# lifthrasiir/j40

Measured on AMD Instinct MI355X. Metric: Mpixels/s RGBA-u8x4 decode, 8K VarDCT d1, higher is better.
Workload: dtype f32

## Files before the change

j40_amd/csrc/device/async.hip:

```cpp
#include <hip/hip_runtime.h>
#include <chrono>
#include <cstdio>
#include <memory>
#include <mutex>
#include <vector>
#include "../decode_route.hpp"
#include "../plan_front.hpp"
#include "kernels.h"
#include "runtime_shared.hpp"
#include "hostcopy.hpp"
#include "async.hpp"

using namespace j40hip;
using namespace j40hip_rt;

namespace {

constexpr uint32_t ERR_GPU = ('!' << 24) | ('g' << 16) | ('p' << 8) | 'u';
constexpr uint32_t ERR_MEM = ('!' << 24) | ('m' << 16) | ('e' << 8) | 'm';

struct StaticEntry {
	int device = 0;
	std::vector<uint8_t> key;
	uint32_t order_off[11 * 13 * 3], dq_off[17], dq_size[17], dq_scan_off[17];
// ... 482 lines not shown
	}
	if ((size_t) n * 4 + 16 > b->verdict_cap) {
		if (b->verdict_host) (void) hipHostFree(b->verdict_host);
		b->verdict_host = nullptr; b->verdict_cap = 0;
		if (hipHostMalloc((void **) &b->verdict_host, 16 * (size_t) n * 2 + 64, hipHostMallocDefault) != hipSuccess) { (void) hipGetLastError(); return ERR_MEM; }
		b->verdict_cap = (size_t) n * 4 * 2 + 16;
	}
	uint8_t *hb = b->host.ptr, *db = (uint8_t *) b->dev;
	b->last_o_k2 = o_k2;
	DevPlan *h_plans = (DevPlan *) (hb + o_plans); DevPlanBuild *h_builds = (DevPlanBuild *) (hb + o_builds); K2Frame *h_k2 = (K2Frame *) (hb + o_k2);
	DevBatchLf *h_lfs = (DevBatchLf *) (hb + o_lfs);
	const DevPlan *d_plans = (const DevPlan *) (db + o_plans); const DevPlanBuild *d_builds = (const DevPlanBuild *) (db + o_builds); K2Frame *d_k2 = (K2Frame *) (db + o_k2);
	const DevBatchLf *d_lfs = (const DevBatchLf *) (db + o_lfs); const HfLaneWork *d_work = (const HfLaneWork *) (db + o_work);
	size_t at_lf = 0;
	for (int i = 0; i < n; ++i) {
		const j40hip_aframe *f = frames[i];
		h_plans[i] = f->plan;
		h_builds[i] = f->build;
		h_builds[i].class_start = d_k2[i].class_start; h_builds[i].verdict = (uint32_t *) (db + o_verdict) + 4 * (size_t) i;
		K2Frame &k = h_k2[i];
		memset(&k, 0, sizeof k);
		k.plan = f->plan; k.sorted = f->build.vb_sorted; k.large_scratch = nullptr; k.rgba = (uint8_t *) rgba_dev[i]; k.stride = stride_bytes[i];
		for (int32_t g = 0; g < f->num_lf_groups; ++g) h_lfs[at_lf++] = DevBatchLf{i, g};
	}
	memcpy(hb + o_work, work.data(), sizeof(HfLaneWork) * work.size());
	if (queue_waves) memcpy(hb + o_queue, queue_start.data(), 4 * queue_start.size());
	if (uint32_t e = wait_for_uploads(frames, n, s)) return e;
	const double tq1 = prof_now();
	if (timing) j40hip_cache_counters(cc1);
	if (hipMemcpyAsync(db, hb, copy_bytes, hipMemcpyHostToDevice, s) != hipSuccess) return ERR_GPU;
	const double tq2 = prof_now();
	launch_clear_block_events(d_plans, d_builds, n, max_frame_cells, s);
	(void) hipEventRecord(b->ev[0], s);
	launch_plan_build(d_builds, d_lfs, n, nlf, max_lf_cells, s);
	launch_lf_tail_batch(d_plans, d_builds, d_lfs, n, nlf, max_lf_cells, max_frame_cells, s);
	for (int i = 0; i < n; ++i) if (!frames[i]->sparse && hipMemsetAsync(frames[i]->plan.coeffs[0], 0, sizeof(float) * 3 * (size_t) frames[i]->plan.coeff_stride, s) != hipSuccess) return ERR_GPU;
	(void) hipEventRecord(b->ev[1], s);
	const double tq3 = prof_now();
	b->k1_timed = lanes_fast;
	if (lanes_fast) launch_hf_lanes(d_plans, d_work, (int32_t) work.size(), waves_per_wg, lanes_lds, s, b->k1_ev[0], b->k1_ev[1], queue_waves ? (uint32_t *) (db + o_queue) : nullptr);
	else launch_hf_entropy_lanes(d_plans, d_work, (int32_t) work.size(), tables_in_lds, generic_lds, s);
	(void) hipEventRecord(b->ev[2], s);
	int32_t grids[K2_NUM_BATCH_LAUNCHES];
	k2_batch_grids(b->have_totals ? b->last_totals : nullptr, cells_total, n, K2_WG_SLOTS, grids);
	launch_vardct_batch(d_k2, n, (int32_t *) (db + o_tiles), (int32_t *) (db + o_verdict + 16 * (size_t) n), grids, b->large_scratch, s, b->side.data(), (int) b->side.size(), b->fork, b->side_done.data(), shift);
	(void) hipEventRecord(b->ev[3], s);
	launch_plan_verdict(d_builds, d_plans, n, s);
	if (hipMemcpyAsync(b->verdict_host, db + o_verdict, 16 * (size_t) n + 64, hipMemcpyDeviceToHost, s) != hipSuccess) return ERR_GPU;
	b->nframes = n; b->have_totals = true;
	if (timing) {
		const double tq4 = prof_now();
		fprintf(stderr, "[j40hip batch launch] bind %.2f (+arrays) %.2f, copy %.2f, plan+tail enqueue %.2f, K1+K2+verdict enqueue %.2f ms; the cache meanwhile (every thread's calls): %llu acquires, %llu hits, %llu + %llu hipMalloc %.2f ms, %llu hipFree %.2f ms, lock %.2f ms, search %.2f ms, %llu idle blocks\n",
			tq1 - tq0, 0.0, tq2 - tq1, tq3 - tq2, tq4 - tq3, (unsigned long long) (cc1[0] - cc0[0]), (unsigned long long) (cc1[1] - cc0[1]), (unsigned long long) (cc1[2] - cc0[2]), (unsigned long long) (cc1[3] - cc0[3]), (double) (cc1[7] - cc0[7]) * 1e-3,
			(unsigned long long) (cc1[4] - cc0[4]), (double) (cc1[8] - cc0[8]) * 1e-3, (double) (cc1[5] - cc0[5]) * 1e-3, (double) (cc1[6] - cc0[6]) * 1e-3, (unsigned long long) cc1[9]);
	}
	return hipGetLastError() == hipSuccess ? 0 : ERR_GPU;
}

uint32_t j40hip_abatch_launch(j40hip_abatch *b, j40hip_aframe *const *frames, int n, void *const *rgba_dev, const size_t *stride_bytes, hipStream_t stream, int32_t shift) {
	if (shift < 0 || shift > 2) return ERR_RNGE;
	try { return abatch_launch_body(b, frames, n, rgba_dev, stride_bytes, stream, shift); } catch (const std::exception &) { return ERR_MEM; }
}

void j40hip_abatch_result(const j40hip_abatch *b, int i, uint32_t *code, int *redo) {
	if (!b || i < 0 || i >= b->nframes) { *code = ERR_GPU; *redo = 0; return; }
	*code = b->verdict_host[4 * (size_t) i]; *redo = b->verdict_host[4 * (size_t) i + 1] != 0;
}

// ... 269 lines not shown
```

j40_amd/csrc/device/kernels.h:

```cpp
#pragma once
#include <hip/hip_runtime.h>
#include "plan.h"
#include "restore_dev.h"
#include "region_dev.h"
#include "colour_dev.h"
#include "patch_dev.h"
#include "noise_dev.h"
#include "spline_dev.h"
#include "upsample_dev.h"

namespace j40hip {

void upload_constant_tables(const float *half_secants, const float *afv_basis, const float *srgb_thr, hipStream_t stream);
void launch_hf_entropy(const DevPlan &plan, const HfLaunchInfo &info, int32_t first_group, int32_t num_groups, hipStream_t stream);
bool hf_entropy_fast_path(const DevPlan &plan, const HfLaunchInfo &info);
void launch_hf_entropy_fast_ordered(const DevPlan &plan, const HfLaunchInfo &info, const uint32_t *order, int32_t first, int32_t count, hipStream_t stream);
void launch_merge_block_events(const DevPlan &plan, const uint32_t *order, int32_t k, const uint32_t *shadow, hipStream_t stream);
void launch_store_group_rects(const uint32_t *order, int32_t k, int32_t gcolumns, int32_t shift, int32_t width, int32_t height, const uint8_t *src, uint8_t *dst_host_mapped, size_t stride_bytes, hipStream_t stream, int32_t pixel_bytes = 4);
uint32_t hf_lanes_lds_bytes(const HfLaunchInfo &info);
void launch_hf_entropy_lanes(const DevPlan *plans, const HfLaneWork *work, int32_t num_work, bool tables_in_lds, uint32_t lds_bytes, hipStream_t stream);
void launch_hf_lanes(const DevPlan *plans, const HfLaneWork *work, int32_t num_work, int32_t waves_per_wg, uint32_t lds_bytes, hipStream_t stream, hipEvent_t started = nullptr, hipEvent_t stopped = nullptr, uint32_t *queue = nullptr);
enum { K2_NUM_BATCH_LAUNCHES = 16, K2_LARGE_WGS = 256, K2_WG_SLOTS = 32768 };
void k2_batch_grids(const int32_t *last_totals, size_t cells_total, int32_t nframes, int32_t wg_slots, int32_t *grids);
void launch_vardct_batch(const K2Frame *frames_dev, int32_t nframes, int32_t *tile_prefix_dev, int32_t *totals_dev, const int32_t *grids, float *large_scratch, hipStream_t stream, hipStream_t *side, int nside, hipEvent_t fork, hipEvent_t *side_done, int32_t shift = 0);
enum class OutMode { RGBA8, XYB, RGBA16, YCC };
struct K2Target { void *base; size_t stride; OutMode out; int32_t shift; };
void launch_vardct_frame(const DevPlan &plan, const int32_t *class_start, const DevVarblock *sorted, float *large_scratch, const K2Target &to, hipStream_t stream);

void launch_epf_sigma(const DevPlan &plan, int32_t num_lf_groups, const int16_t *sharpness, const RestoreParams &p, float *sigma, uint32_t *sharp_or, hipStream_t stream);
void launch_epf_sigma_cells(const int16_t *sharpness, const float *hfmul_inv, const RestoreParams &p, float *sigma, uint32_t *sharp_or, hipStream_t stream);
float *launch_restoration(float *xyb, float *tmp, size_t pitch, const RestoreParams &p, bool gab, int32_t epf_iters, const float *sigma, hipStream_t stream);
void launch_xyb_to_rgba(const float *xyb, size_t pitch, const DevFrame *frame_dev, int32_t width, int32_t height, uint8_t *rgba, size_t stride_bytes, hipStream_t stream, bool rgba16 = false);

void launch_colour_tail(const float *xyb, size_t pitch, const ColourTailParams &p, int32_t width, int32_t height, uint8_t *out, size_t stride_bytes, hipStream_t stream, bool rgba16 = false);

void launch_patch_blend(float *planes, int32_t width, int32_t height, const DevPatches &p, const PatchSlots &slots, hipStream_t stream);

void launch_noise_fill(float *raw, const NoiseFillArgs &a, const uint64_t *sets_dev, hipStream_t stream);
void launch_noise_add(float *planes, size_t ppitch, const float *raw, int32_t W, int32_t H, const NoiseParams &p, hipStream_t stream);

bool launch_upsample(const float *src, int32_t w, int32_t h, int32_t k, const float *table_dev, float *out, int32_t up_w, int32_t up_h, hipStream_t stream);

void launch_spline_draw(float *planes, size_t pitch, int32_t W, int32_t H, const DevSplines &d, hipStream_t stream);

void upload_lf_tail_tables(const float *half_secants, const float *lf2llf, hipStream_t stream);
void launch_lf_tail(const DevPlan &plan, int32_t num_lf_groups, int32_t max_cells, size_t cells, float *lfs, const DevVarblock *sorted, int32_t count, int32_t first_large, int32_t smooth,
		const float inv_m_lf[3], hipStream_t stream);
void launch_lf_frame_tail(const DevPlan &plan, int32_t num_lf_groups, int32_t max_cells, size_t cells, float *lfs, const DevVarblock *sorted, int32_t count, int32_t first_large,
		LfFrameArgs args, bool bctx, int32_t num_groups, hipStream_t stream);

void launch_lf_tail_batch(const DevPlan *plans, const DevPlanBuild *builds, const DevBatchLf *lfs, int32_t nframes, int32_t nlf, int32_t max_lf_cells, size_t max_frame_cells, hipStream_t stream);
void launch_plan_build(const DevPlanBuild *builds, const DevBatchLf *lfs, int32_t nframes, int32_t nlf, int32_t max_lf_cells, hipStream_t stream);
void launch_clear_block_events(const DevPlan *plans, const DevPlanBuild *builds, int32_t nframes, size_t max_frame_cells, hipStream_t stream);
void launch_plan_verdict(const DevPlanBuild *builds, const DevPlan *plans, int32_t nframes, hipStream_t stream);

enum { LFP_U8 = 0, LFP_U16 = 1, LFP_PLANE = 2, LFP_LANES = 256 };
void upload_lf_preview_tables(const float *srgb_thr, hipStream_t stream);
void launch_lf_preview(const DevLfpFrame *frames, const DevLfpWork *work, int32_t nwork, uint32_t nblocks, int32_t mode, int32_t channel, hipStream_t stream);

void launch_kat_srgb_u8(const float *v, size_t n, uint8_t *out, hipStream_t stream);
void launch_kat_srgb_u16(const float *v, size_t n, int32_t bpp, uint16_t *out, hipStream_t stream);

void launch_modular_sections(const DevModPlan &plan, int32_t first_section, int32_t num_sections, const ModLaunchInfo &info, hipStream_t stream);
void launch_lf_groups(const DevLfTask *tasks, int32_t num_tasks, hipStream_t stream);
#include <vector>
uint32_t pack_lf_waves(const DevLfLaneSet *sets_host, int32_t num_sets, std::vector<DevLfWave> *waves, const std::vector<int32_t> *only = nullptr);
void launch_lf_lanes(const DevLfLaneSet *sets, const DevLfWave *waves, int32_t num_waves, uint32_t lds_bytes, hipStream_t stream, hipEvent_t started = nullptr, hipEvent_t stopped = nullptr);
bool lf_rows_enabled();
uint32_t pack_lf_row_waves(const DevLfLaneSet *sets_host, int32_t num_sets, std::vector<DevLfWave> *waves, std::vector<int32_t> *oversized = nullptr);
void launch_lf_rows(const DevLfLaneSet *sets, const DevLfWave *waves, int32_t num_waves, uint32_t lds_bytes, hipStream_t stream, hipEvent_t started = nullptr, hipEvent_t stopped = nullptr);
void launch_modular_quad(const DevModPlan &plan, int32_t first_section, int32_t num_sections, int32_t spec_idx, uint32_t table_span, int32_t max_width, hipStream_t stream);
void launch_modular_split(const DevModPlan &plan, int32_t first_section, int32_t num_sections, const ModLaunchInfo &info, hipStream_t stream);
void launch_modular_coop(const DevModPlan &plan, int32_t first_section, int32_t num_sections, int32_t max_width, hipStream_t stream, bool wide = false);
void launch_section_inverse_rcts(const DevModPlan &plan, int32_t first_section, int32_t num_sections, hipStream_t stream, bool wide = false);
void launch_paste_plane(PlanePtr src, int32_t w, int32_t h, PlanePtr dst, int32_t dst_stride, hipStream_t stream);
void launch_inverse_rct(PlanePtr a, PlanePtr b, PlanePtr c, size_t n, int32_t type7, hipStream_t stream);
void launch_inverse_palette_plain(PlanePtr idx, PlanePtr palrow, PlanePtr dst, size_t n, int32_t i, int32_t nb_colours, int32_t bpp, hipStream_t stream);
void launch_inverse_palette_predicted(PlanePtr idx, PlanePtr pal, int32_t pal_stride, void *const *dst_dev, int32_t num_c, int32_t width, int32_t height,
		int32_t nb_colours, int32_t nb_deltas, int32_t d_pred, int32_t bpp, const int8_t *wpp_dev, int32_t *wp_scratch, uint32_t *status, hipStream_t stream);
void launch_inverse_squeeze(PlanePtr avg, PlanePtr res, PlanePtr out, int32_t aw, int32_t ah, int32_t rw, int32_t rh, bool horizontal, hipStream_t stream);
void launch_pack_planes_rect(PlanePtr r, PlanePtr g, PlanePtr b, PlanePtr a, int32_t plane_width, int32_t x0, int32_t y0, int32_t rw, int32_t rh, int32_t bpp, uint8_t *rgba, size_t stride, hipStream_t stream, bool rgba16 = false);
void launch_alpha_merge(const int16_t *plane, int32_t pitch, int32_t x0, int32_t y0, int32_t w, int32_t h, int32_t bpp, uint8_t *rgba, size_t stride, hipStream_t stream, bool rgba16);
struct YcbcrTail;
void launch_ycbcr_tail(const YcbcrTail &t, uint8_t *rgba, size_t stride, hipStream_t stream, bool rgba16);
void launch_pack_planes(PlanePtr r, PlanePtr g, PlanePtr b, PlanePtr a, int32_t width, int32_t height, int32_t bpp, uint8_t *rgba, size_t stride, hipStream_t stream, bool rgba16 = false, int32_t shift = 0);
// ... 23 lines not shown
```

j40_amd/csrc/device/lf_tail_kernels.hip:

```cpp
#include <hip/hip_runtime.h>
#include "hf_dev.h"
#include "lf_smooth_dev.h"
#include "lf_frame_dev.h"
#include "kernels.h"

namespace j40hip {

__constant__ float c_tail_half_secants[256];
__constant__ float c_tail_lf2llf[64];

void upload_lf_tail_tables(const float *half_secants, const float *lf2llf, hipStream_t stream) {
	(void) hipMemcpyToSymbolAsync(HIP_SYMBOL(c_tail_half_secants), half_secants, sizeof(float) * 256, 0, hipMemcpyHostToDevice, stream);
	(void) hipMemcpyToSymbolAsync(HIP_SYMBOL(c_tail_lf2llf), lf2llf, sizeof(float) * 64, 0, hipMemcpyHostToDevice, stream);
}

__device__ __forceinline__ void lf_dequant_smooth_cell(const DevPlan &plan, const DevLfGroup &gg, int32_t i, float *out0, float *out1, float *out2, int32_t smooth, float inv0, float inv1, float inv2) {
	const int32_t w8 = gg.width8, h8 = gg.height8;
	if (i >= w8 * h8) return;
	const int32_t y = i / w8, x = i - y * w8;
	const size_t at = (size_t) gg.cell_base + (size_t) i;
	float *out[3] = {out0, out1, out2};
	const float inv_m_lf[3] = {inv0, inv1, inv2};
	const bool edge = !smooth || w8 < 3 || h8 < 3 || y == 0 || x == 0 || y == h8 - 1 || x == w8 - 1;
	if (edge) {
// ... 74 lines not shown
	if (R * C > 1) llf_block<LR, LC>(buf);
#pragma unroll
	for (int k = 0; k < R * C; ++k) llf[k] = buf[k];
}

__device__ __forceinline__ void llf_small_one(const DevPlan &plan, const DevVarblock &vb, const float *lf0, const float *lf1, const float *lf2, float *llf0, float *llf1, float *llf2) {
	const int32_t log_rows = DEV_DCT_SELECT[vb.dctsel][0], log_columns = DEV_DCT_SELECT[vb.dctsel][1];
	if (log_rows > 5 || log_columns > 5) return;
	const DevLfGroup gg = plan.lf_groups[(uint32_t) vb.pad[0] | ((uint32_t) vb.pad[1] << 8) | ((uint32_t) vb.pad[2] << 16)];
	const size_t cell = (size_t) gg.cell_base + (size_t) ((vb.py - gg.top) >> 3) * (size_t) gg.width8 + (size_t) ((vb.px - gg.left) >> 3);
	const float *lf[3] = {lf0, lf1, lf2};
	float *llf[3] = {llf0, llf1, llf2};
	for (int c = 0; c < 3; ++c) {
		float *dst = llf[c] + vb.llf_base;
		switch ((log_rows - 3) * 3 + (log_columns - 3)) {
		case 0: llf_small_case<0, 0>(lf[c], cell, gg.width8, dst); break;
		case 1: llf_small_case<0, 1>(lf[c], cell, gg.width8, dst); break;
		case 2: llf_small_case<0, 2>(lf[c], cell, gg.width8, dst); break;
		case 3: llf_small_case<1, 0>(lf[c], cell, gg.width8, dst); break;
		case 4: llf_small_case<1, 1>(lf[c], cell, gg.width8, dst); break;
		case 5: llf_small_case<1, 2>(lf[c], cell, gg.width8, dst); break;
		case 6: llf_small_case<2, 0>(lf[c], cell, gg.width8, dst); break;
		case 7: llf_small_case<2, 1>(lf[c], cell, gg.width8, dst); break;
		default: llf_small_case<2, 2>(lf[c], cell, gg.width8, dst); break;
		}
	}
}

__global__ void __launch_bounds__(256) k_llf_small(DevPlan plan, const DevVarblock *list, int32_t count, const float *lf0, const float *lf1, const float *lf2, float *llf0, float *llf1, float *llf2) {
	const int32_t v = (int32_t) (blockIdx.x * blockDim.x + threadIdx.x);
	if (v >= count) return;
	llf_small_one(plan, list[v], lf0, lf1, lf2, llf0, llf1, llf2);
}
__global__ void __launch_bounds__(256) k_llf_small_batch(const DevPlan *plans, const DevPlanBuild *builds) {
	const DevPlan &plan = plans[blockIdx.y];
	const DevPlanBuild &pb = builds[blockIdx.y];
	const int32_t v = (int32_t) (blockIdx.x * blockDim.x + threadIdx.x);
	if (v >= pb.class_start[27]) return;
	const float *lfs = pb.lf_scratch;
	llf_small_one(plan, pb.vb_sorted[v], lfs, lfs + pb.cells, lfs + 2 * (size_t) pb.cells, const_cast<float *>(plan.llf[0]), const_cast<float *>(plan.llf[1]), const_cast<float *>(plan.llf[2]));
}

__device__ void fwd_dct_rt(float *out, float *in, int32_t t, int32_t stride) {
	const int32_t N = 1 << t;
	if (t == 0) { out[0] = in[0]; return; }
	if (t == 1) { const float x = in[0], y = in[stride]; out[0] = x + y; out[stride] = x - y; return; }
	for (int32_t i = 0; i < N / 2; ++i) {
		const float x = in[i * stride], y = in[(N - i - 1) * stride];
		out[i * stride] = x + y;
		out[(N / 2 + i) * stride] = (x - y) * c_tail_half_secants[N / 2 + i];
	}
	fwd_dct_rt(in, out, t - 1, stride);
	fwd_dct_rt(in + N / 2 * stride, out + N / 2 * stride, t - 1, stride);
	for (int32_t i = 0; i < N / 2; ++i) out[i * 2 * stride] = in[i * stride];
	out[stride] = 1.4142135623730951f * in[N / 2 * stride] + in[(N / 2 + 1) * stride];
	for (int32_t i = 1; i < N / 2 - 1; ++i) out[(i * 2 + 1) * stride] = in[(N / 2 + i) * stride] + in[(N / 2 + i + 1) * stride];
	out[(N - 1) * stride] = in[(N - 1) * stride];
}

__device__ void llf_large_one(const DevPlan &plan, const DevVarblock &vb, const float *lf0, const float *lf1, const float *lf2, float *llf0, float *llf1, float *llf2, float *buf, float *tmp, int32_t lane) {
	const int32_t lr = DEV_DCT_SELECT[vb.dctsel][0] - 3, lc = DEV_DCT_SELECT[vb.dctsel][1] - 3, R = 1 << lr, C = 1 << lc;
	const DevLfGroup gg = plan.lf_groups[(uint32_t) vb.pad[0] | ((uint32_t) vb.pad[1] << 8) | ((uint32_t) vb.pad[2] << 16)];
	const size_t cell = (size_t) gg.cell_base + (size_t) ((vb.py - gg.top) >> 3) * (size_t) gg.width8 + (size_t) ((vb.px - gg.left) >> 3);
	const float *lf[3] = {lf0, lf1, lf2};
	float *llf[3] = {llf0, llf1, llf2};
	for (int c = 0; c < 3; ++c) {
		for (int32_t k = lane; k < R * C; k += 64) buf[k] = lf[c][cell + (size_t) (k / C) * (size_t) gg.width8 + (size_t) (k % C)];
		__syncthreads();
		for (int32_t r = lane; r < C; r += 64) fwd_dct_rt(tmp + r, buf + r, lr, C);
		__syncthreads();
		for (int32_t k = lane; k < R * C; k += 64) { const int32_t y = k / C, x = k % C; buf[x * R + y] = tmp[y * C + x]; }
		__syncthreads();
		for (int32_t r = lane; r < R; r += 64) fwd_dct_rt(tmp + r, buf + r, lc, R);
// ... 22 lines not shown
		llf_large_one(plan, pb.vb_sorted[v], lfs, lfs + pb.cells, lfs + 2 * (size_t) pb.cells, const_cast<float *>(plan.llf[0]), const_cast<float *>(plan.llf[1]), const_cast<float *>(plan.llf[2]), buf, tmp, threadIdx.x);
}

__global__ void __launch_bounds__(256) k_lf_from_frame(DevPlan plan, LfFrameArgs args) {
	lf_from_frame_cell(plan.lf_groups[blockIdx.y], (int32_t) (blockIdx.x * blockDim.x + threadIdx.x), args);
}
__global__ void __launch_bounds__(256) k_lf_frame_bctx(DevPlan plan, DevGroupBlock *blocks, const uint8_t *lfindices) {
	lf_frame_bctx_block(plan, blocks, lfindices, (int32_t) blockIdx.y, blockIdx.x * blockDim.x + threadIdx.x);
}

static void launch_llf(const DevPlan &plan, size_t cells, float *lfs, const DevVarblock *sorted, int32_t count, int32_t first_large, hipStream_t stream) {
	float *llf0 = const_cast<float *>(plan.llf[0]), *llf1 = const_cast<float *>(plan.llf[1]), *llf2 = const_cast<float *>(plan.llf[2]);
	if (count > 0) hipLaunchKernelGGL(k_llf_small, dim3((unsigned) ((count + 255) / 256)), dim3(256), 0, stream, plan, sorted, count, lfs, lfs + cells, lfs + 2 * cells, llf0, llf1, llf2);
	if (count > first_large) hipLaunchKernelGGL(k_llf_large, dim3((unsigned) (count - first_large)), dim3(64), 0, stream, plan, sorted + first_large, count - first_large, lfs, lfs + cells, lfs + 2 * cells, llf0, llf1, llf2);
}

void launch_lf_tail(const DevPlan &plan, int32_t num_lf_groups, int32_t max_cells, size_t cells, float *lfs, const DevVarblock *sorted, int32_t count, int32_t first_large, int32_t smooth,
		const float inv_m_lf[3], hipStream_t stream) {
	if (num_lf_groups <= 0 || max_cells <= 0) return;
	hipLaunchKernelGGL(k_lf_dequant_smooth, dim3((unsigned) ((max_cells + 255) / 256), (unsigned) num_lf_groups), dim3(256), 0, stream, plan, lfs, lfs + cells, lfs + 2 * cells, smooth, inv_m_lf[0], inv_m_lf[1], inv_m_lf[2]);
	launch_llf(plan, cells, lfs, sorted, count, first_large, stream);
}

void launch_lf_frame_tail(const DevPlan &plan, int32_t num_lf_groups, int32_t max_cells, size_t cells, float *lfs, const DevVarblock *sorted, int32_t count, int32_t first_large,
		LfFrameArgs args, bool bctx, int32_t num_groups, hipStream_t stream) {
	if (num_lf_groups <= 0 || max_cells <= 0) return;
	args.out[0] = lfs; args.out[1] = lfs + cells; args.out[2] = lfs + 2 * cells;
	args.lfindices = const_cast<uint8_t *>(plan.lfindices);
	hipLaunchKernelGGL(k_lf_from_frame, dim3((unsigned) ((max_cells + 255) / 256), (unsigned) num_lf_groups), dim3(256), 0, stream, plan, args);
	if (bctx && num_groups > 0) hipLaunchKernelGGL(k_lf_frame_bctx, dim3(4, (unsigned) num_groups), dim3(256), 0, stream, plan, const_cast<DevGroupBlock *>(plan.group_blocks), plan.lfindices);
	launch_llf(plan, cells, lfs, sorted, count, first_large, stream);
}

void launch_lf_tail_batch(const DevPlan *plans, const DevPlanBuild *builds, const DevBatchLf *lfs, int32_t nframes, int32_t nlf, int32_t max_lf_cells, size_t max_frame_cells, hipStream_t stream) {
	if (nframes <= 0 || nlf <= 0 || max_lf_cells <= 0) return;
	hipLaunchKernelGGL(k_lf_dequant_smooth_batch, dim3((unsigned) ((max_lf_cells + 255) / 256), (unsigned) nlf), dim3(256), 0, stream, plans, builds, lfs);
	hipLaunchKernelGGL(k_llf_small_batch, dim3((unsigned) ((max_frame_cells + 255) / 256), (unsigned) nframes), dim3(256), 0, stream, plans, builds);
	hipLaunchKernelGGL(k_llf_large_batch, dim3(32, (unsigned) nframes), dim3(64), 0, stream, plans, builds);
}

}
```

j40_amd/csrc/device/plan_dev.h:

```cpp
#pragma once
#include "hf_dev.h"
#include "lf_frame_dev.h"

namespace j40hip {

enum { PLAN_LOG_GSIZE8 = 5 };

J40_DEV void plan_place_lf_group(const DevPlanBuild &pb, int32_t g, uint16_t *occ, uint16_t *grp_cnt, uint32_t *cls_cnt, int32_t stride) {
	DevLfGroup &gg = pb.lf_groups[g];
	DevLfSlot &slot = pb.lf_slots[g];
	const int32_t w8 = gg.width8, h8 = gg.height8;
	const int32_t ggx = g % pb.ggcolumns, ggy = g / pb.ggcolumns;
	for (int32_t x = 0; x < w8; ++x) occ[x * stride] = 0;
	for (int32_t i = 0; i < 64; ++i) grp_cnt[i * stride] = 0;
	for (int32_t i = 0; i < 28; ++i) cls_cnt[i * stride] = 0;
	uint32_t err = slot.status, used = 0;
	int32_t voff = 0;
	if (!err) {
		const int32_t nbv = slot.nb_varblocks;
		const int16_t *info0 = pb.vbinfo + 2 * (size_t) gg.cell_base, *info1 = info0 + nbv;
		DevVbRec *recs = pb.vb_recs + gg.vb_base;
		const int32_t coeff_limit = w8 * h8 * 64;
		int32_t coeffoff = 0;
		for (int32_t y0 = 0; y0 < h8 && !err; ++y0) for (int32_t x0 = 0; x0 < w8; ++x0) {
// ... 51 lines not shown
	const uint32_t blk = pb.group_block_start[gid] + r.rank_in_group;
	const size_t cell = (size_t) gg.cell_base + (size_t) y8 * (size_t) gg.width8 + (size_t) x8;
	uint8_t lfidx = 0;
	{
		const int32_t vx = pb.lfraw[0][cell], vy = pb.lfraw[1][cell], vb = pb.lfraw[2][cell];
		for (int32_t t = 0; t < pb.nb_lf_thr[0]; ++t) lfidx = (uint8_t) (lfidx + (vx > pb.lf_thr[0][t]));
		lfidx = (uint8_t) (lfidx * (pb.nb_lf_thr[0] + 1));
		for (int32_t t = 0; t < pb.nb_lf_thr[2]; ++t) lfidx = (uint8_t) (lfidx + (vb > pb.lf_thr[2][t]));
		lfidx = (uint8_t) (lfidx * (pb.nb_lf_thr[2] + 1));
		for (int32_t t = 0; t < pb.nb_lf_thr[1]; ++t) lfidx = (uint8_t) (lfidx + (vy > pb.lf_thr[1][t]));
	}
	const int32_t log_rows = DEV_DCT_SELECT[dctsel][0], log_columns = DEV_DCT_SELECT[dctsel][1], order_idx = DEV_DCT_SELECT[dctsel][2];
	DevGroupBlock gb;
	gb.coeffoff_qfidx = r.coeffoff_qfidx;
	gb.pos_dct = (uint16_t) (((y8 & 31) * 32 + (x8 & 31)) | (dctsel << 10));
	gb.bctx3 = (uint16_t) block_ctx3(pb.pool_u8 + pb.block_ctx_map_off, order_idx, (int32_t) (r.coeffoff_qfidx & 15u), lfidx, pb.nb_qf_thr + 1, pb.lfidx_size);
	pb.group_blocks[blk] = gb;
	DevVarblock dv;
	const int32_t coeffoff = (int32_t) (r.coeffoff_qfidx & ~15u);
	dv.coeff_base = gg.cell_base * 64 + coeffoff; dv.llf_base = gg.cell_base + (coeffoff >> 6);
	dv.mult1 = pb.mult_base * (1.0f / ((float) r.hfmul_m1 + 1.0f));
	const size_t c64 = (size_t) gg.c64_base + (size_t) (y8 / 8) * (size_t) gg.width64 + (size_t) (x8 / 8);
	dv.kx_hf = pb.base_corr_x + pb.inv_colour_factor * (float) pb.xfromy[c64];
	dv.kb_hf = pb.base_corr_b + pb.inv_colour_factor * (float) pb.bfromy[c64];
	dv.px = gg.left + x8 * 8; dv.py = gg.top + y8 * 8;
	const int32_t eh = gg.height - y8 * 8, ew = gg.width - x8 * 8;
	dv.effh = (uint16_t) (eh < (1 << log_rows) ? eh : 1 << log_rows); dv.effw = (uint16_t) (ew < (1 << log_columns) ? ew : 1 << log_columns);
	dv.dctsel = (uint8_t) dctsel;
	dv.pad[0] = (uint8_t) g; dv.pad[1] = (uint8_t) (g >> 8); dv.pad[2] = (uint8_t) (g >> 16);
	dv.blk = (int32_t) blk;
	pb.vb_sorted[pb.class_count[g * 28 + dctsel] + r.rank_in_class] = dv;
}

J40_DEV uint64_t plan_verdict_key(uint32_t status, uint32_t byte_off) { return status && status != (uint32_t) ERR_LFFB ? (uint64_t) byte_off << 32 | status : ~(uint64_t) 0; }

}
```

j40_amd/csrc/device/plan_kernels.hip:

```cpp
#include <hip/hip_runtime.h>
#include "plan_dev.h"
#include "kernels.h"
#include "../env.hpp"
#include <climits>
#include <algorithm>

namespace j40hip {

__global__ void __launch_bounds__(64) k_plan_place_lanes(const DevPlanBuild *builds, const DevBatchLf *lfs, int32_t nlf) {
	__shared__ uint16_t occ[256 * 64];
	__shared__ uint16_t grp[64 * 64];
	__shared__ uint32_t cls[28 * 64];
	const int32_t i = (int32_t) (blockIdx.x * 64 + threadIdx.x);
	if (i >= nlf) return;
	const DevBatchLf w = lfs[i];
	plan_place_lf_group(builds[w.frame], w.lfg, occ + threadIdx.x, grp + threadIdx.x, cls + threadIdx.x, 64);
}

__device__ __forceinline__ int32_t pp_rl(int32_t v, int32_t lane) { return __builtin_amdgcn_readlane(v, lane); }
__device__ __forceinline__ int32_t pp_sc(int32_t v) { return __builtin_amdgcn_readfirstlane(v); }

__global__ void __launch_bounds__(64) k_plan_place_walk(const DevPlanBuild *builds, const DevBatchLf *lfs, int32_t nlf) {
	const int32_t lane = threadIdx.x;
	const DevBatchLf w = lfs[blockIdx.x];
// ... 42 lines not shown
						if (q == 0) occ0 = mine && occ0 < below ? below : occ0; else if (q == 1) occ1 = mine && occ1 < below ? below : occ1;
						else if (q == 2) occ2 = mine && occ2 < below ? below : occ2; else occ3 = mine && occ3 < below ? below : occ3;
					}
					const int32_t qf = (int32_t) __builtin_popcountll(__builtin_amdgcn_ballot_w64(lane < nb_qf_thr && hfmul_m1 >= my_thr));
					const int32_t grp = (y0 >> PLAN_LOG_GSIZE8) * 8 + (x0 >> PLAN_LOG_GSIZE8);
					const int32_t rank_g = pp_rl(grp_cnt, grp), rank_c = pp_rl(cls_cnt, dctsel);
					grp_cnt += lane == grp; cls_cnt += lane == dctsel;
					if (lane == (voff & 63)) {
						r0 = (uint32_t) (coeffoff + qf);
						r1 = (uint32_t) (uint16_t) (int16_t) hfmul_m1 | (uint32_t) x0 << 16 | (uint32_t) y0 << 24;
						r2 = (uint32_t) dctsel | (uint32_t) grp << 8 | (uint32_t) rank_g << 16;
						r3 = (uint32_t) rank_c;
					}
					used |= 1u << dctsel;
					coeffoff += 1 << (log_rows + log_columns);
					++voff;
					if ((voff & 63) == 0) ((uint4 *) recs)[voff - 64 + lane] = make_uint4(r0, r1, r2, r3);
				}
			}
		}
		if ((voff & 63) != 0 && lane < (voff & 63)) ((uint4 *) recs)[(voff & ~63) + lane] = make_uint4(r0, r1, r2, r3);
		if (!err && voff != nbv) err = ERR_VBLK;
	}
	if (lane == 0) { slot->status = err; slot->placed = voff; slot->dct_used = used; ggp->nb_varblocks = voff; }
	{
		const int32_t gx = lane & 7, gy = lane >> 3;
		if ((gx << PLAN_LOG_GSIZE8) < w8 && (gy << PLAN_LOG_GSIZE8) < h8) pb.group_count[(ggy * 8 + gy) * pb.gcolumns + ggx * 8 + gx] = (uint32_t) grp_cnt;
	}
	if (lane < 28) pb.class_count[g * 28 + lane] = lane < 27 ? (uint32_t) cls_cnt : 0u;
}

__device__ __forceinline__ int32_t pp_below(uint64_t m) { return (int32_t) __builtin_amdgcn_mbcnt_hi((uint32_t) (m >> 32), __builtin_amdgcn_mbcnt_lo((uint32_t) m, 0u)); }

__global__ void __launch_bounds__(64) k_plan_place(const DevPlanBuild *builds, const DevBatchLf *lfs, int32_t nlf) {
	const int32_t lane = threadIdx.x;
	const DevBatchLf w = lfs[blockIdx.x];
	const DevPlanBuild &pb = builds[w.frame];
	const int32_t g = w.lfg;
	DevLfGroup *ggp = pb.lf_groups + g;
	DevLfSlot *slot = pb.lf_slots + g;
	const int32_t w8 = pp_sc(ggp->width8), h8 = pp_sc(ggp->height8), cell_base = pp_sc(ggp->cell_base), vb_base = pp_sc(ggp->vb_base);
	const int32_t ggx = g % pb.ggcolumns, ggy = g / pb.ggcolumns;
	uint32_t err = (uint32_t) pp_sc((int32_t) slot->status), used = 0;
	const int32_t nbv = pp_sc(slot->nb_varblocks), nb_qf_thr = pp_sc(pb.nb_qf_thr);
	const int32_t my_thr = lane < nb_qf_thr ? pb.qf_thr[lane < 15 ? lane : 14] : 0;
	const int32_t my_dims = lane < 27 ? (int32_t) DEV_DCT_SELECT[lane][0] | ((int32_t) DEV_DCT_SELECT[lane][1] << 8) : 0;
	int32_t occ0 = 0, occ1 = 0, occ2 = 0, occ3 = 0;
	int32_t grp_cnt = 0, cls_cnt = 0;
	int32_t voff = 0;
	if (!err) {
		const int16_t *info0 = pb.vbinfo + 2 * (size_t) cell_base, *info1 = info0 + nbv;
		DevVbRec *recs = pb.vb_recs + vb_base;
		const int32_t coeff_limit = w8 * h8 * 64;
		int32_t coeffoff = 0;
		int32_t chunk_coeffoff = 0;
		int32_t chunk = -1, i0 = 0, i1 = 0;
		int32_t pos = 0;
		auto records = [&](int32_t first, int32_t n) {
			const bool valid = lane < n;
			const int32_t dctsel = valid ? i0 : 0, hfmul_m1 = i1;
			const int32_t dims = __builtin_amdgcn_ds_bpermute(dctsel << 2, my_dims);
			const int32_t size = valid ? 1 << ((dims & 255) + (dims >> 8)) : 0;
			int32_t upto = size;
			for (int32_t d = 1; d < 64; d <<= 1) { const int32_t o = __shfl_up(upto, d); upto += lane >= d ? o : 0; }
			const int32_t my_off = chunk_coeffoff + upto - size;
			chunk_coeffoff += pp_rl(upto, 63);
			int32_t qf = 0;
			for (int32_t t = 0; t < nb_qf_thr; ++t) qf += hfmul_m1 >= pp_rl(my_thr, t) ? 1 : 0;
			const int32_t x0 = pos & 255, y0 = (pos >> 8) & 255;
			const int32_t grp = (y0 >> PLAN_LOG_GSIZE8) * 8 + (x0 >> PLAN_LOG_GSIZE8);
			int32_t rank_g = __builtin_amdgcn_ds_bpermute(grp << 2, grp_cnt), rank_c = __builtin_amdgcn_ds_bpermute(dctsel << 2, cls_cnt);
			for (uint64_t todo = __builtin_amdgcn_ballot_w64(valid); todo; ) {
				const int32_t key = pp_rl(grp, (int32_t) __builtin_ctzll(todo));
				const uint64_t same = __builtin_amdgcn_ballot_w64(valid && grp == key);
				rank_g += valid && grp == key ? pp_below(same) : 0;
				grp_cnt += lane == key ? (int32_t) __builtin_popcountll(same) : 0;
				todo &= ~same;
			}
			for (uint64_t todo = __builtin_amdgcn_ballot_w64(valid); todo; ) {
				const int32_t key = pp_rl(dctsel, (int32_t) __builtin_ctzll(todo));
				const uint64_t same = __builtin_amdgcn_ballot_w64(valid && dctsel == key);
				rank_c += valid && dctsel == key ? pp_below(same) : 0;
				cls_cnt += lane == key ? (int32_t) __builtin_popcountll(same) : 0;
				todo &= ~same;
			}
			if (valid) ((uint4 *) recs)[first + lane] = make_uint4((uint32_t) (my_off + qf), (uint32_t) (uint16_t) (int16_t) hfmul_m1 | (uint32_t) x0 << 16 | (uint32_t) y0 << 24,
				(uint32_t) dctsel | (uint32_t) grp << 8 | (uint32_t) rank_g << 16, (uint32_t) rank_c);
		};
		for (int32_t y0 = 0; y0 < h8 && !err; ++y0) {
			for (int32_t q = 0; q < 4 && !err; ++q) {
				if (q * 64 >= w8) break;
				const int32_t occq = q == 0 ? occ0 : q == 1 ? occ1 : q == 2 ? occ2 : occ3;
				uint64_t free_mask = __builtin_amdgcn_ballot_w64(occq <= y0 && q * 64 + lane < w8);
				while (free_mask) {
					const int32_t bit = (int32_t) __builtin_ctzll(free_mask), x0 = q * 64 + bit;
					if (voff >= nbv) { err = ERR_VBLK; break; }
					if ((voff >> 6) != chunk) {
						chunk = voff >> 6;
						const int32_t k = chunk * 64 + lane;
						i0 = k < nbv ? (int32_t) info0[k] : 0; i1 = k < nbv ? (int32_t) info1[k] : 0;
					}
					const int32_t dctsel = pp_rl(i0, voff & 63);
					if (dctsel < 0 || dctsel >= 27) { err = ERR_DCTQ; break; }
					const int32_t dims = pp_rl(my_dims, dctsel), log_rows = dims & 255, log_columns = dims >> 8;
					const int32_t vw8 = 1 << (log_columns - 3), vh8 = 1 << (log_rows - 3), x1 = x0 + vw8 - 1, y1 = y0 + vh8 - 1;
					if (!(x1 < w8 && (x0 >> PLAN_LOG_GSIZE8) == (x1 >> PLAN_LOG_GSIZE8)) || !(y1 < h8 && (y0 >> PLAN_LOG_GSIZE8) == (y1 >> PLAN_LOG_GSIZE8))) { err = ERR_VBLK; break; }
					if (coeffoff + (1 << (log_rows + log_columns)) > coeff_limit) { err = ERR_VBLK; break; }
					free_mask &= ~((((uint64_t) 1 << vw8) - 1) << bit);
					if (vh8 > 1) {
						const bool mine = lane >= bit && lane < bit + vw8;
						const int32_t below = y1 + 1;
						if (q == 0) occ0 = mine && occ0 < below ? below : occ0; else if (q == 1) occ1 = mine && occ1 < below ? below : occ1;
						else if (q == 2) occ2 = mine && occ2 < below ? below : occ2; else occ3 = mine && occ3 < below ? below : occ3;
					}
					pos = lane == (voff & 63) ? x0 | y0 << 8 : pos;
					used |= 1u << dctsel;
					coeffoff += 1 << (log_rows + log_columns);
					++voff;
					if ((voff & 63) == 0) records(voff - 64, 64);
				}
			}
		}
		if ((voff & 63) != 0) records(voff & ~63, voff & 63);
		if (!err && voff != nbv) err = ERR_VBLK;
	}
	if (lane == 0) { slot->status = err; slot->placed = voff; slot->dct_used = used; ggp->nb_varblocks = voff; }
	{
		const int32_t gx = lane & 7, gy = lane >> 3;
		if ((gx << PLAN_LOG_GSIZE8) < w8 && (gy << PLAN_LOG_GSIZE8) < h8) pb.group_count[(ggy * 8 + gy) * pb.gcolumns + ggx * 8 + gx] = (uint32_t) grp_cnt;
	}
	if (lane < 28) pb.class_count[g * 28 + lane] = lane < 27 ? (uint32_t) cls_cnt : 0u;
}

__global__ void __launch_bounds__(64) k_plan_scan(const DevPlanBuild *builds, int32_t nframes) {
	const int32_t f = (int32_t) (blockIdx.x * 64 + threadIdx.x);
	if (f < nframes) plan_scan_frame(builds[f]);
}

__global__ void __launch_bounds__(256) k_plan_emit(const DevPlanBuild *builds, const DevBatchLf *lfs) {
	const DevBatchLf w = lfs[blockIdx.y];
	const DevPlanBuild &pb = builds[w.frame];
	const int32_t v = (int32_t) (blockIdx.x * 256 + threadIdx.x);
	if (v < pb.lf_slots[w.lfg].placed) plan_emit_varblock(pb, w.lfg, v);
}

__global__ void __launch_bounds__(64) k_plan_verdict(const DevPlanBuild *builds, const DevPlan *plans) {
	const DevPlanBuild &pb = builds[blockIdx.x];
	const DevPlan &plan = plans[blockIdx.x];
	const int32_t lane = threadIdx.x, nsec = plan.frame->num_passes * pb.num_groups;
	uint64_t best = ~(uint64_t) 0;
	uint32_t flags = 0, used = 0;
	for (int32_t g = lane; g < pb.num_lf_groups; g += 64) {
		const DevLfSlot sl = pb.lf_slots[g];
		if (sl.status == (uint32_t) ERR_LFFB) flags |= 1u;
		used |= sl.dct_used;
		const uint64_t k = plan_verdict_key(sl.status, pb.lf_section_off[g]);
		best = k < best ? k : best;
	}
	for (int32_t i = lane; i < nsec; i += 64) {
		const uint32_t st = plan.status[i];
		if (st == (uint32_t) ERR_EVOF) flags |= 2u;
		const uint64_t k = plan_verdict_key(st, plan.sections[i].byte_off);
		best = k < best ? k : best;
	}
	for (int d = 32; d >= 1; d >>= 1) {
		const uint64_t o = __shfl_xor(best, d);
		best = o < best ? o : best;
		flags |= __shfl_xor(flags, d); used |= __shfl_xor(used, d);
	}
	if (lane == 0) { pb.verdict[0] = best == ~(uint64_t) 0 ? 0u : (uint32_t) best; pb.verdict[1] = flags; pb.verdict[2] = used; pb.verdict[3] = (uint32_t) pb.class_start[27]; }
}

__global__ void __launch_bounds__(256) k_clear_block_events(const DevPlan *plans, const DevPlanBuild *builds) {
	const DevPlan &plan = plans[blockIdx.y];
	if (!plan.block_events) return;
	const uint32_t cells = builds[blockIdx.y].cells;
	uint4 *p = (uint4 *) plan.block_events;
	for (uint32_t i = blockIdx.x * 256u + threadIdx.x; i < cells; i += gridDim.x * 256u) p[i] = make_uint4(0, 0, 0, 0);
}
void launch_clear_block_events(const DevPlan *plans, const DevPlanBuild *builds, int32_t nframes, size_t max_frame_cells, hipStream_t stream) {
	if (nframes <= 0 || !max_frame_cells) return;
	const unsigned gx = (unsigned) std::min<size_t>((max_frame_cells + 255) / 256, 256);
	hipLaunchKernelGGL(k_clear_block_events, dim3(gx, (unsigned) nframes), dim3(256), 0, stream, plans, builds);
}

void launch_plan_build(const DevPlanBuild *builds, const DevBatchLf *lfs, int32_t nframes, int32_t nlf, int32_t max_lf_cells, hipStream_t stream) {
	if (nframes <= 0 || nlf <= 0) return;
	static const bool lanes_form = env_on("J40HIP_PLAN_PLACE_LANES", false);
	static const int form = env_int("J40HIP_PLAN_PLACE_FORM", 0, INT_MIN, INT_MAX);
	if (lanes_form) hipLaunchKernelGGL(k_plan_place_lanes, dim3((unsigned) ((nlf + 63) / 64)), dim3(64), 0, stream, builds, lfs, nlf);
	else if (form == 1) hipLaunchKernelGGL(k_plan_place_walk, dim3((unsigned) nlf), dim3(64), 0, stream, builds, lfs, nlf);
	else hipLaunchKernelGGL(k_plan_place, dim3((unsigned) nlf), dim3(64), 0, stream, builds, lfs, nlf);
	hipLaunchKernelGGL(k_plan_scan, dim3((unsigned) ((nframes + 63) / 64)), dim3(64), 0, stream, builds, nframes);
	hipLaunchKernelGGL(k_plan_emit, dim3((unsigned) ((max_lf_cells + 255) / 256), (unsigned) nlf), dim3(256), 0, stream, builds, lfs);
}

void launch_plan_verdict(const DevPlanBuild *builds, const DevPlan *plans, int32_t nframes, hipStream_t stream) {
	if (nframes > 0) hipLaunchKernelGGL(k_plan_verdict, dim3((unsigned) nframes), dim3(64), 0, stream, builds, plans);
}

}
```

Before: 12610.

## Fuse one-cell LLF into plan emit and batch runs of 8x8 blocks in placement

LF dequant/smooth is moved ahead of plan building so that plan_emit can also write LLF values for single-cell (8x8) varblocks. This removes those blocks from the small-LLF kernel, which now walks only classes 4..11 with a fixed grid-stride launch. Plan placement gains a run-based fast path that places consecutive 8x8 varblocks a wave at a time through a shared cell table. It derives the used-DCT mask from class counts. The cost is extra per-emit work and more complex placement logic.

```diff
diff --git a/j40_amd/csrc/device/async.hip b/j40_amd/csrc/device/async.hip
--- a/j40_amd/csrc/device/async.hip
+++ b/j40_amd/csrc/device/async.hip
@@ -538,8 +538,9 @@
 	const double tq2 = prof_now();
 	launch_clear_block_events(d_plans, d_builds, n, max_frame_cells, s);
 	(void) hipEventRecord(b->ev[0], s);
-	launch_plan_build(d_builds, d_lfs, n, nlf, max_lf_cells, s);
-	launch_lf_tail_batch(d_plans, d_builds, d_lfs, n, nlf, max_lf_cells, max_frame_cells, s);
+	launch_lf_dequant_smooth_batch(d_plans, d_builds, d_lfs, n, nlf, max_lf_cells, s);
+	launch_plan_build(d_builds, d_plans, d_lfs, n, nlf, max_lf_cells, s);
+	launch_llf_batch(d_plans, d_builds, n, nlf, max_lf_cells, s);
 	for (int i = 0; i < n; ++i) if (!frames[i]->sparse && hipMemsetAsync(frames[i]->plan.coeffs[0], 0, sizeof(float) * 3 * (size_t) frames[i]->plan.coeff_stride, s) != hipSuccess) return ERR_GPU;
 	(void) hipEventRecord(b->ev[1], s);
 	const double tq3 = prof_now();
diff --git a/j40_amd/csrc/device/kernels.h b/j40_amd/csrc/device/kernels.h
--- a/j40_amd/csrc/device/kernels.h
+++ b/j40_amd/csrc/device/kernels.h
@@ -49,8 +49,9 @@
 void launch_lf_frame_tail(const DevPlan &plan, int32_t num_lf_groups, int32_t max_cells, size_t cells, float *lfs, const DevVarblock *sorted, int32_t count, int32_t first_large,
 		LfFrameArgs args, bool bctx, int32_t num_groups, hipStream_t stream);
 
-void launch_lf_tail_batch(const DevPlan *plans, const DevPlanBuild *builds, const DevBatchLf *lfs, int32_t nframes, int32_t nlf, int32_t max_lf_cells, size_t max_frame_cells, hipStream_t stream);
-void launch_plan_build(const DevPlanBuild *builds, const DevBatchLf *lfs, int32_t nframes, int32_t nlf, int32_t max_lf_cells, hipStream_t stream);
+void launch_lf_dequant_smooth_batch(const DevPlan *plans, const DevPlanBuild *builds, const DevBatchLf *lfs, int32_t nframes, int32_t nlf, int32_t max_lf_cells, hipStream_t stream);
+void launch_llf_batch(const DevPlan *plans, const DevPlanBuild *builds, int32_t nframes, int32_t nlf, int32_t max_lf_cells, hipStream_t stream);
+void launch_plan_build(const DevPlanBuild *builds, const DevPlan *plans, const DevBatchLf *lfs, int32_t nframes, int32_t nlf, int32_t max_lf_cells, hipStream_t stream);
 void launch_clear_block_events(const DevPlan *plans, const DevPlanBuild *builds, int32_t nframes, size_t max_frame_cells, hipStream_t stream);
 void launch_plan_verdict(const DevPlanBuild *builds, const DevPlan *plans, int32_t nframes, hipStream_t stream);
 
diff --git a/j40_amd/csrc/device/lf_tail_kernels.hip b/j40_amd/csrc/device/lf_tail_kernels.hip
--- a/j40_amd/csrc/device/lf_tail_kernels.hip
+++ b/j40_amd/csrc/device/lf_tail_kernels.hip
@@ -130,13 +130,14 @@
 	if (v >= count) return;
 	llf_small_one(plan, list[v], lf0, lf1, lf2, llf0, llf1, llf2);
 }
+enum { LLF_SMALL_BATCH_WGS = 64 };
 __global__ void __launch_bounds__(256) k_llf_small_batch(const DevPlan *plans, const DevPlanBuild *builds) {
 	const DevPlan &plan = plans[blockIdx.y];
 	const DevPlanBuild &pb = builds[blockIdx.y];
-	const int32_t v = (int32_t) (blockIdx.x * blockDim.x + threadIdx.x);
-	if (v >= pb.class_start[27]) return;
 	const float *lfs = pb.lf_scratch;
-	llf_small_one(plan, pb.vb_sorted[v], lfs, lfs + pb.cells, lfs + 2 * (size_t) pb.cells, const_cast<float *>(plan.llf[0]), const_cast<float *>(plan.llf[1]), const_cast<float *>(plan.llf[2]));
+	const int32_t end = pb.class_start[12];
+	for (int32_t v = pb.class_start[4] + (int32_t) (blockIdx.x * blockDim.x + threadIdx.x); v < end; v += (int32_t) (gridDim.x * blockDim.x))
+		llf_small_one(plan, pb.vb_sorted[v], lfs, lfs + pb.cells, lfs + 2 * (size_t) pb.cells, const_cast<float *>(plan.llf[0]), const_cast<float *>(plan.llf[1]), const_cast<float *>(plan.llf[2]));
 }
 
 __device__ void fwd_dct_rt(float *out, float *in, int32_t t, int32_t stride) {
@@ -225,10 +226,13 @@
 	launch_llf(plan, cells, lfs, sorted, count, first_large, stream);
 }
 
-void launch_lf_tail_batch(const DevPlan *plans, const DevPlanBuild *builds, const DevBatchLf *lfs, int32_t nframes, int32_t nlf, int32_t max_lf_cells, size_t max_frame_cells, hipStream_t stream) {
+void launch_lf_dequant_smooth_batch(const DevPlan *plans, const DevPlanBuild *builds, const DevBatchLf *lfs, int32_t nframes, int32_t nlf, int32_t max_lf_cells, hipStream_t stream) {
 	if (nframes <= 0 || nlf <= 0 || max_lf_cells <= 0) return;
 	hipLaunchKernelGGL(k_lf_dequant_smooth_batch, dim3((unsigned) ((max_lf_cells + 255) / 256), (unsigned) nlf), dim3(256), 0, stream, plans, builds, lfs);
-	hipLaunchKernelGGL(k_llf_small_batch, dim3((unsigned) ((max_frame_cells + 255) / 256), (unsigned) nframes), dim3(256), 0, stream, plans, builds);
+}
+void launch_llf_batch(const DevPlan *plans, const DevPlanBuild *builds, int32_t nframes, int32_t nlf, int32_t max_lf_cells, hipStream_t stream) {
+	if (nframes <= 0 || nlf <= 0 || max_lf_cells <= 0) return;
+	hipLaunchKernelGGL(k_llf_small_batch, dim3(LLF_SMALL_BATCH_WGS, (unsigned) nframes), dim3(256), 0, stream, plans, builds);
 	hipLaunchKernelGGL(k_llf_large_batch, dim3(32, (unsigned) nframes), dim3(64), 0, stream, plans, builds);
 }
 
diff --git a/j40_amd/csrc/device/plan_dev.h b/j40_amd/csrc/device/plan_dev.h
--- a/j40_amd/csrc/device/plan_dev.h
+++ b/j40_amd/csrc/device/plan_dev.h
@@ -107,6 +107,19 @@
 	pb.vb_sorted[pb.class_count[g * 28 + dctsel] + r.rank_in_class] = dv;
 }
 
+J40_DEV bool plan_one_cell(int32_t dctsel) { return DEV_DCT_SELECT[dctsel][0] == 3 && DEV_DCT_SELECT[dctsel][1] == 3; }
+
+J40_DEV void plan_emit_llf_one_cell(const DevPlanBuild &pb, int32_t g, int32_t v, float *llf0, float *llf1, float *llf2) {
+	const DevLfGroup &gg = pb.lf_groups[g];
+	const DevVbRec r = pb.vb_recs[gg.vb_base + v];
+	if (!plan_one_cell(r.dctsel)) return;
+	const size_t cell = (size_t) gg.cell_base + (size_t) r.y8 * (size_t) gg.width8 + (size_t) r.x8;
+	const size_t llf_base = (size_t) (gg.cell_base + (int32_t) ((r.coeffoff_qfidx & ~15u) >> 6));
+	llf0[llf_base] = pb.lf_scratch[cell];
+	llf1[llf_base] = pb.lf_scratch[(size_t) pb.cells + cell];
+	llf2[llf_base] = pb.lf_scratch[2 * (size_t) pb.cells + cell];
+}
+
 J40_DEV uint64_t plan_verdict_key(uint32_t status, uint32_t byte_off) { return status && status != (uint32_t) ERR_LFFB ? (uint64_t) byte_off << 32 | status : ~(uint64_t) 0; }
 
 }
diff --git a/j40_amd/csrc/device/plan_kernels.hip b/j40_amd/csrc/device/plan_kernels.hip
--- a/j40_amd/csrc/device/plan_kernels.hip
+++ b/j40_amd/csrc/device/plan_kernels.hip
@@ -98,7 +98,12 @@
 
 __device__ __forceinline__ int32_t pp_below(uint64_t m) { return (int32_t) __builtin_amdgcn_mbcnt_hi((uint32_t) (m >> 32), __builtin_amdgcn_mbcnt_lo((uint32_t) m, 0u)); }
 
-__global__ void __launch_bounds__(64) k_plan_place(const DevPlanBuild *builds, const DevBatchLf *lfs, int32_t nlf) {
+#ifndef J40_PLAN_PLACE_MIN_RUN
+#define J40_PLAN_PLACE_MIN_RUN 1
+#endif
+enum { PLAN_PLACE_MIN_RUN = J40_PLAN_PLACE_MIN_RUN };
+
+template <bool RUNS> __device__ __forceinline__ void plan_place_wave(const DevPlanBuild *builds, const DevBatchLf *lfs, int32_t *cell_of) {
 	const int32_t lane = threadIdx.x;
 	const DevBatchLf w = lfs[blockIdx.x];
 	const DevPlanBuild &pb = builds[w.frame];
@@ -122,6 +127,7 @@
 		int32_t chunk_coeffoff = 0;
 		int32_t chunk = -1, i0 = 0, i1 = 0;
 		int32_t pos = 0;
+		uint64_t one = 0;
 		auto records = [&](int32_t first, int32_t n) {
 			const bool valid = lane < n;
 			const int32_t dctsel = valid ? i0 : 0, hfmul_m1 = i1;
@@ -165,6 +171,33 @@
 						chunk = voff >> 6;
 						const int32_t k = chunk * 64 + lane;
 						i0 = k < nbv ? (int32_t) info0[k] : 0; i1 = k < nbv ? (int32_t) info1[k] : 0;
+						if (RUNS) {
+							const bool known = k < nbv && i0 >= 0 && i0 < 27;
+							const int32_t dims = __builtin_amdgcn_ds_bpermute((known ? i0 : 0) << 2, my_dims);
+							one = __builtin_amdgcn_ballot_w64(known & (dims == (3 | 3 << 8)));
+						}
+					}
+					if (RUNS) {
+						const int32_t p = voff & 63;
+						const uint64_t stop = ~(one >> p);
+						int32_t n = stop ? (int32_t) __builtin_ctzll(stop) : 64;
+						n = min(n, (int32_t) __builtin_popcountll(free_mask));
+						n = min(n, (coeff_limit - coeffoff) >> 6);
+						if (n >= PLAN_PLACE_MIN_RUN) {
+							const bool is_free = (free_mask >> lane) & 1;
+							const int32_t rank = pp_below(free_mask);
+							if (is_free && rank < n) cell_of[p + rank] = (q * 64 + lane) | y0 << 8;
+							__builtin_amdgcn_fence(__ATOMIC_RELEASE, "workgroup");
+							__builtin_amdgcn_wave_barrier();
+							__builtin_amdgcn_fence(__ATOMIC_ACQUIRE, "workgroup");
+							const int32_t got = cell_of[lane];
+							pos = lane >= p && lane < p + n ? got : pos;
+							free_mask = __builtin_amdgcn_ballot_w64(is_free && rank >= n);
+							coeffoff += 64 * n;
+							voff += n;
+							if ((voff & 63) == 0) records(voff - 64, 64);
+							continue;
+						}
 					}
 					const int32_t dctsel = pp_rl(i0, voff & 63);
 					if (dctsel < 0 || dctsel >= 27) { err = ERR_DCTQ; break; }
@@ -180,7 +213,7 @@
 						else if (q == 2) occ2 = mine && occ2 < below ? below : occ2; else occ3 = mine && occ3 < below ? below : occ3;
 					}
 					pos = lane == (voff & 63) ? x0 | y0 << 8 : pos;
-					used |= 1u << dctsel;
+					if (!RUNS) used |= 1u << dctsel;
 					coeffoff += 1 << (log_rows + log_columns);
 					++voff;
 					if ((voff & 63) == 0) records(voff - 64, 64);
@@ -188,6 +221,7 @@
 			}
 		}
 		if ((voff & 63) != 0) records(voff & ~63, voff & 63);
+		if (RUNS) used = (uint32_t) __builtin_amdgcn_ballot_w64(cls_cnt != 0) & 0x7ffffffu;
 		if (!err && voff != nbv) err = ERR_VBLK;
 	}
 	if (lane == 0) { slot->status = err; slot->placed = voff; slot->dct_used = used; ggp->nb_varblocks = voff; }
@@ -198,16 +232,29 @@
 	if (lane < 28) pb.class_count[g * 28 + lane] = lane < 27 ? (uint32_t) cls_cnt : 0u;
 }
 
+__global__ void __launch_bounds__(64) k_plan_place(const DevPlanBuild *builds, const DevBatchLf *lfs, int32_t nlf) {
+	__shared__ int32_t cell_of[64];
+	(void) nlf;
+	plan_place_wave<true>(builds, lfs, cell_of);
+}
+__global__ void __launch_bounds__(64) k_plan_place_blocks(const DevPlanBuild *builds, const DevBatchLf *lfs, int32_t nlf) {
+	(void) nlf;
+	plan_place_wave<false>(builds, lfs, nullptr);
+}
+
 __global__ void __launch_bounds__(64) k_plan_scan(const DevPlanBuild *builds, int32_t nframes) {
 	const int32_t f = (int32_t) (blockIdx.x * 64 + threadIdx.x);
 	if (f < nframes) plan_scan_frame(builds[f]);
 }
 
-__global__ void __launch_bounds__(256) k_plan_emit(const DevPlanBuild *builds, const DevBatchLf *lfs) {
+__global__ void __launch_bounds__(256) k_plan_emit(const DevPlanBuild *builds, const DevPlan *plans, const DevBatchLf *lfs) {
 	const DevBatchLf w = lfs[blockIdx.y];
 	const DevPlanBuild &pb = builds[w.frame];
+	const DevPlan &plan = plans[w.frame];
 	const int32_t v = (int32_t) (blockIdx.x * 256 + threadIdx.x);
-	if (v < pb.lf_slots[w.lfg].placed) plan_emit_varblock(pb, w.lfg, v);
+	if (v >= pb.lf_slots[w.lfg].placed) return;
+	plan_emit_varblock(pb, w.lfg, v);
+	plan_emit_llf_one_cell(pb, w.lfg, v, const_cast<float *>(plan.llf[0]), const_cast<float *>(plan.llf[1]), const_cast<float *>(plan.llf[2]));
 }
 
 __global__ void __launch_bounds__(64) k_plan_verdict(const DevPlanBuild *builds, const DevPlan *plans) {
@@ -250,15 +297,16 @@
 	hipLaunchKernelGGL(k_clear_block_events, dim3(gx, (unsigned) nframes), dim3(256), 0, stream, plans, builds);
 }
 
-void launch_plan_build(const DevPlanBuild *builds, const DevBatchLf *lfs, int32_t nframes, int32_t nlf, int32_t max_lf_cells, hipStream_t stream) {
+void launch_plan_build(const DevPlanBuild *builds, const DevPlan *plans, const DevBatchLf *lfs, int32_t nframes, int32_t nlf, int32_t max_lf_cells, hipStream_t stream) {
 	if (nframes <= 0 || nlf <= 0) return;
 	static const bool lanes_form = env_on("J40HIP_PLAN_PLACE_LANES", false);
 	static const int form = env_int("J40HIP_PLAN_PLACE_FORM", 0, INT_MIN, INT_MAX);
 	if (lanes_form) hipLaunchKernelGGL(k_plan_place_lanes, dim3((unsigned) ((nlf + 63) / 64)), dim3(64), 0, stream, builds, lfs, nlf);
 	else if (form == 1) hipLaunchKernelGGL(k_plan_place_walk, dim3((unsigned) nlf), dim3(64), 0, stream, builds, lfs, nlf);
+	else if (form == 2) hipLaunchKernelGGL(k_plan_place_blocks, dim3((unsigned) nlf), dim3(64), 0, stream, builds, lfs, nlf);
 	else hipLaunchKernelGGL(k_plan_place, dim3((unsigned) nlf), dim3(64), 0, stream, builds, lfs, nlf);
 	hipLaunchKernelGGL(k_plan_scan, dim3((unsigned) ((nframes + 63) / 64)), dim3(64), 0, stream, builds, nframes);
-	hipLaunchKernelGGL(k_plan_emit, dim3((unsigned) ((max_lf_cells + 255) / 256), (unsigned) nlf), dim3(256), 0, stream, builds, lfs);
+	hipLaunchKernelGGL(k_plan_emit, dim3((unsigned) ((max_lf_cells + 255) / 256), (unsigned) nlf), dim3(256), 0, stream, builds, plans, lfs);
 }
 
 void launch_plan_verdict(const DevPlanBuild *builds, const DevPlan *plans, int32_t nframes, hipStream_t stream) {
```

Result: no change. 12630, median of 2 (+0.2%).
